# PathologyFoundation/plip

Measured on NVIDIA H100. Metric: image-text pairs/sec (224x224, 77-tok), higher is better.
Workload: dtype bf16

## Files before the change

plip_b200/csrc/attention.cu:

```cuda
#include <cfloat>

#include "kernels.cuh"
#include "wgmma.cuh"

namespace plip {

namespace {

constexpr int kAttThreads = 256;
constexpr uint32_t kTileBytes = 128 * 64 * 2;
constexpr uint32_t kStageBytes = 3 * kTileBytes;
constexpr uint32_t kAttSmem = kStageBytes + 1024 + 64;

__device__ __forceinline__ float fast_exp2(float x) {
  float y;
  asm("ex2.approx.ftz.f32 %0, %1;" : "=f"(y) : "f"(x));
  return y;
}
constexpr float kLog2e = 1.4426950408889634f;


template <bool F16, int NK>
__device__ __forceinline__ void qk_scores(float (&s)[NK / 2], uint64_t qdesc, uint64_t kdesc) {
  wgmma_pin(s);
  wgmma_fence();
#pragma unroll
  for (int k = 0; k < kHeadDim / 16; ++k) {
    if constexpr (NK == 64) wgmma_ss_n64<F16>(s, qdesc + 2 * k, kdesc + 2 * k, k != 0 ? 1u : 0u);
    else wgmma_ss_n128<F16>(s, qdesc + 2 * k, kdesc + 2 * k, k != 0 ? 1u : 0u);
  }
  wgmma_commit();
  wgmma_wait<0>();
  wgmma_pin(s);
}

__device__ __forceinline__ void quad_max(float& a, float& b) {
#pragma unroll
  for (int o = 1; o < 4; o <<= 1) {
    a = fmaxf(a, __shfl_xor_sync(0xffffffffu, a, o));
    b = fmaxf(b, __shfl_xor_sync(0xffffffffu, b, o));
  }
}
__device__ __forceinline__ void quad_sum(float& a, float& b) {
#pragma unroll
  for (int o = 1; o < 4; o <<= 1) {
    a += __shfl_xor_sync(0xffffffffu, a, o);
    b += __shfl_xor_sync(0xffffffffu, b, o);
  }
}

__device__ __forceinline__ int last_visible_key(int row, int S, int causal) {
  return row < S ? (causal ? row : S - 1) : -1;
}

template <int N>
__device__ __forceinline__ void mask_column(float (&s)[N], int j, int e, bool ok, int key, int lim0, int lim1) {
  if (!(ok && key <= lim0)) s[4 * j + e] = -INFINITY;
  if (!(ok && key <= lim1)) s[4 * j + 2 + e] = -INFINITY;
}

__device__ __forceinline__ float row_shift(float m) { return fmaxf(m * kLog2e, -FLT_MAX); }
__device__ __forceinline__ float row_inv(float l) { return l > 0.f ? 1.0f / l : 0.f; }

__device__ __forceinline__ float softmax_exp(float s, float ms) { return fast_exp2(fmaf(s, kLog2e, -ms)); }

__device__ __forceinline__ float2 fold_row_max(const float (&s)[32], float& m0, float& m1, float& l0, float& l1) {
  float mx0 = m0, mx1 = m1;
#pragma unroll
  for (int j = 0; j < 8; ++j) {
    mx0 = fmaxf(mx0, fmaxf(s[4 * j + 0], s[4 * j + 1]));
    mx1 = fmaxf(mx1, fmaxf(s[4 * j + 2], s[4 * j + 3]));
  }
  quad_max(mx0, mx1);
  const float alpha0 = softmax_exp(m0, row_shift(mx0)), alpha1 = softmax_exp(m1, row_shift(mx1));
  m0 = mx0;
  m1 = mx1;
  l0 *= alpha0;
  l1 *= alpha1;
  return make_float2(alpha0, alpha1);
}

template <bool F16, int N>
__device__ __forceinline__ void exp_sum_pack(const float (&s)[N], float ms0, float ms1, float& l0, float& l1,
                                             uint32_t (&pa)[N / 8][4]) {
#pragma unroll
  for (int j = 0; j < N / 4; ++j) {
    const float e00 = softmax_exp(s[4 * j + 0], ms0), e01 = softmax_exp(s[4 * j + 1], ms0);
    const float e10 = softmax_exp(s[4 * j + 2], ms1), e11 = softmax_exp(s[4 * j + 3], ms1);
    l0 += e00 + e01;
    l1 += e10 + e11;
    pa[j >> 1][2 * (j & 1) + 0] = pack_op2<F16>(e00, e01);
    pa[j >> 1][2 * (j & 1) + 1] = pack_op2<F16>(e10, e11);
  }
}

template <bool F16>
__device__ __forceinline__ void stage_rows(uint32_t row0, const float (&o)[32], float inv0, float inv1, int rr, int q4) {
  const uint32_t row1 = row0 + 8u * 128u;
#pragma unroll
  for (int j = 0; j < 8; ++j) {
    st_shared_b32(row0 + ((j ^ rr) << 4) + q4 * 4, pack_op2<F16>(o[4 * j + 0] * inv0, o[4 * j + 1] * inv0));
    st_shared_b32(row1 + ((j ^ rr) << 4) + q4 * 4, pack_op2<F16>(o[4 * j + 2] * inv1, o[4 * j + 3] * inv1));
  }
}

struct AttParams {
  int64_t n_seq;
  int seq_len;
  int slot;
  int group;
  int heads;
  int64_t seq_tiles;
  int causal;
  const int32_t* key_mask;
};

template <bool F16, int NK>
__global__ void __launch_bounds__(kAttThreads, NK == 64 ? 3 : 2)
attention_kernel(const __grid_constant__ CUtensorMap tmLoad, const __grid_constant__ CUtensorMap tmStore,
                 const AttParams p) {
  extern __shared__ uint8_t smem_raw[];
  const uint32_t smem_base = (smem_u32(smem_raw) + 1023u) & ~1023u;
  const uint32_t bar = smem_base + kStageBytes;
  const uint32_t sq = smem_base, sk = smem_base + kTileBytes, sv = smem_base + 2 * kTileBytes;

  const int warp = threadIdx.x >> 5;
  const int lane = threadIdx.x & 31;
  const int hf = warp >> 2;
  const int D = p.heads * kHeadDim;
  const int S = p.seq_len, G = p.group, slot = p.slot;

  if (threadIdx.x == 0) {
    tma_prefetch_desc(&tmLoad);
    tma_prefetch_desc(&tmStore);
    mbar_init(bar, 1);
    fence_mbar_init();
  }
  __syncthreads();

  const int ntiles = (int)(p.seq_tiles * p.heads);
  const uint32_t slot_bytes = static_cast<uint32_t>(slot) * 128u;
  auto issue_loads = [&](int tile) {
    const int64_t st = tile / p.heads;
    const int h = (int)(tile - st * p.heads);
    mbar_arrive_expect_tx(bar, 3 * kTileBytes);
    for (int g = 0; g < G; ++g) {
      const int32_t row = (int32_t)((st * G + g) * S);
      tma_load_2d(sq + g * slot_bytes, &tmLoad, bar, h * kHeadDim, row);
      tma_load_2d(sk + g * slot_bytes, &tmLoad, bar, D + h * kHeadDim, row);
      tma_load_2d(sv + g * slot_bytes, &tmLoad, bar, 2 * D + h * kHeadDim, row);
    }
  };
  if (threadIdx.x == 0 && (int)blockIdx.x < ntiles) issue_loads(blockIdx.x);

  const int q4 = lane & 3, rr = lane >> 2;
  const int R0 = 64 * hf + 16 * (warp & 3) + rr;
  const int g = R0 / slot;
  const int r_in0 = R0 - g * slot, r_in1 = r_in0 + 8;
  const int kbase = (NK == 64) ? 64 * hf : 0;
  const int k_in_base = kbase - g * slot + 2 * q4;
  const int lim0 = last_visible_key(r_in0, S, p.causal), lim1 = last_visible_key(r_in1, S, p.causal);

  uint32_t it = 0;
  for (int tile = blockIdx.x; tile < ntiles; tile += gridDim.x, ++it) {
    const int st = tile / p.heads;
    const int h = tile - st * p.heads;
    const int64_t seq = (int64_t)st * G + g;

    uint32_t kv = 0;
#pragma unroll
    for (int c = 0; c < NK / 4; ++c) {
      const int k_in = k_in_base + 8 * (c >> 1) + (c & 1);
      bool ok = k_in >= 0 && k_in < S;
      if (ok && p.key_mask != nullptr) ok = seq < p.n_seq && p.key_mask[seq * S + k_in] != 0;
      kv |= (ok ? 1u : 0u) << c;
    }

    mbar_wait(bar, it & 1u);

    float s[NK / 2];
    qk_scores<F16, NK>(s, make_smem_desc_sw128(sq + hf * (64 * 128), 1024, 16),
                       make_smem_desc_sw128(sk + kbase * 128, 1024, 16));

    float mx0 = -INFINITY, mx1 = -INFINITY;
#pragma unroll
    for (int c = 0; c < NK / 4; ++c) {
      const int j = c >> 1, e = c & 1;
      mask_column(s, j, e, (kv >> c) & 1u, k_in_base + 8 * j + e, lim0, lim1);
      mx0 = fmaxf(mx0, s[4 * j + e]);
      mx1 = fmaxf(mx1, s[4 * j + 2 + e]);
    }
    quad_max(mx0, mx1);
    float sum0 = 0.f, sum1 = 0.f;
    uint32_t pa[NK / 16][4];
    exp_sum_pack<F16>(s, row_shift(mx0), row_shift(mx1), sum0, sum1, pa);
    quad_sum(sum0, sum1);

    float o[32];
    wgmma_pin(o);
    wgmma_fence();
#pragma unroll
    for (int kk = 0; kk < NK / 16; ++kk) {
      const uint64_t vdesc = make_smem_desc_sw128(sv + (kbase + 16 * kk) * 128, 1024, 1024);
      wgmma_rs_n64<F16>(o, pa[kk], vdesc, kk != 0 ? 1u : 0u);
    }
    wgmma_commit();
    wgmma_wait<0>();
    wgmma_pin(o);

    stage_rows<F16>(sq + static_cast<uint32_t>(R0) * 128u, o, row_inv(sum0), row_inv(sum1), rr, q4);
    fence_proxy_async_smem();
    __syncthreads();
    if (threadIdx.x == 0) {
      for (int gg = 0; gg < G; ++gg) {
        const int64_t sq_idx = (int64_t)st * G + gg;
        if (sq_idx < p.n_seq)
          tma_store_2d(&tmStore, sq + static_cast<uint32_t>(gg * slot) * 128u, h * kHeadDim, (int32_t)(sq_idx * S));
      }
      tma_store_commit();
      tma_store_wait_read();
      if (tile + (int)gridDim.x < ntiles) issue_loads(tile + gridDim.x);
    }
  }
  if (threadIdx.x == 0) tma_store_wait_all();
}

template <bool F16, int NK>
int launch_attention_inst(const CUtensorMap& tmL, const CUtensorMap& tmS, const AttParams& p, cudaStream_t st) {
  auto kern = attention_kernel<F16, NK>;
  static unsigned long long configured = 0;
  static int grid_cap = 0;
  if (first_use_on_device(configured)) {
    PLIP_CUDA_CHECK(cudaFuncSetAttribute(kern, cudaFuncAttributeMaxDynamicSharedMemorySize, (int)kAttSmem));
    int dev = 0, sms = 0, per_sm = 0;
    PLIP_CUDA_CHECK(cudaGetDevice(&dev));
    PLIP_CUDA_CHECK(cudaDeviceGetAttribute(&sms, cudaDevAttrMultiProcessorCount, dev));
    PLIP_CUDA_CHECK(cudaOccupancyMaxActiveBlocksPerMultiprocessor(&per_sm, kern, kAttThreads, kAttSmem));
    grid_cap = (per_sm > 0 ? per_sm : 1) * sms;
  }
  const int64_t tiles = p.seq_tiles * p.heads;
  const int grid = (int)(tiles < grid_cap ? tiles : grid_cap);
  PLIP_CUDA_CHECK(launch_kernel(kern, dim3(grid), dim3(kAttThreads), kAttSmem, st, 1, tmL, tmS, p));
  return 0;
}

constexpr int kLongThreads = 288;
constexpr int kLongKeys = 64;
constexpr uint32_t kLongQBytes = 128 * 64 * 2;
constexpr uint32_t kLongKVBytes = kLongKeys * 64 * 2;
constexpr int kLongStages = 2;
constexpr uint32_t kLongSmem = kLongQBytes + kLongStages * 2 * kLongKVBytes + 1024 + 64;

struct LongAttParams {
  int seq_len;
  int heads;
  int q_blocks;
};

template <bool F16>
__global__ void __launch_bounds__(kLongThreads, 2)
attention_long_kernel(const __grid_constant__ CUtensorMap tmQKV, const __grid_constant__ CUtensorMap tmO,
                      const LongAttParams p) {
  extern __shared__ uint8_t smem_raw[];
  const uint32_t smem_base = (smem_u32(smem_raw) + 1023u) & ~1023u;
  const uint32_t sq = smem_base;
  auto sk = [&](int s) { return smem_base + kLongQBytes + (uint32_t)s * 2u * kLongKVBytes; };
  auto sv = [&](int s) { return sk(s) + kLongKVBytes; };
  const uint32_t bar = smem_base + kLongQBytes + kLongStages * 2 * kLongKVBytes;
  const uint32_t q_bar = bar;
  auto full_bar = [&](int s) { return bar + 8u * (1 + s); };
  auto empty_bar = [&](int s) { return bar + 8u * (1 + kLongStages + s); };

  const int warp = threadIdx.x >> 5;
  const int lane = threadIdx.x & 31;
  const int wg = warp >> 2;
  const int S = p.seq_len, D = p.heads * kHeadDim;
  const int qb = blockIdx.x % p.q_blocks;
  const int bh = blockIdx.x / p.q_blocks;
  const int h = bh % p.heads;
  const int seq = bh / p.heads;
  const int q0 = qb * 128;
  const int n_kb = (S + kLongKeys - 1) / kLongKeys;

  if (threadIdx.x == 0) {
    tma_prefetch_desc(&tmQKV);
    tma_prefetch_desc(&tmO);
    mbar_init(q_bar, 1);
    for (int s = 0; s < kLongStages; ++s) {
      mbar_init(full_bar(s), 1);
      mbar_init(empty_bar(s), 2);
    }
    fence_mbar_init();
  }
  __syncthreads();

  if (wg == 2) {
    if (lane == 0) {
      mbar_arrive_expect_tx(q_bar, kLongQBytes);
      tma_load_3d(sq, &tmQKV, q_bar, h * kHeadDim, q0, seq);
      tma_load_3d(sq + kLongQBytes / 2, &tmQKV, q_bar, h * kHeadDim, q0 + 64, seq);
      for (int kb = 0; kb < n_kb; ++kb) {
        const int s = kb % kLongStages;
        if (kb >= kLongStages) mbar_wait(empty_bar(s), (uint32_t)((kb / kLongStages - 1) & 1));
        mbar_arrive_expect_tx(full_bar(s), 2 * kLongKVBytes);
        tma_load_3d(sk(s), &tmQKV, full_bar(s), D + h * kHeadDim, kb * kLongKeys, seq);
        tma_load_3d(sv(s), &tmQKV, full_bar(s), 2 * D + h * kHeadDim, kb * kLongKeys, seq);
      }
    }
    return;
  }

  const int q4 = lane & 3, rr = lane >> 2;
  const int R0 = 64 * wg + 16 * (warp & 3) + rr;
  float o[32];
#pragma unroll
  for (int i = 0; i < 32; ++i) o[i] = 0.f;
  float m0 = -INFINITY, m1 = -INFINITY;
  float l0 = 0.f, l1 = 0.f;
  const uint64_t qdesc = make_smem_desc_sw128(sq + wg * (64 * 128), 1024, 16);
  mbar_wait(q_bar, 0);

  for (int kb = 0; kb < n_kb; ++kb) {
    const int s = kb % kLongStages;
    mbar_wait(full_bar(s), (uint32_t)((kb / kLongStages) & 1));

    float sc[32];
    qk_scores<F16, 64>(sc, qdesc, make_smem_desc_sw128(sk(s), 1024, 16));

    const int kbase = kb * kLongKeys + 2 * q4;
    if (kb * kLongKeys + kLongKeys > S) {
#pragma unroll
      for (int j = 0; j < 8; ++j)
#pragma unroll
        for (int e = 0; e < 2; ++e)
          if (kbase + 8 * j + e >= S) {
            sc[4 * j + e] = -INFINITY;
            sc[4 * j + 2 + e] = -INFINITY;
          }
    }
    const float2 alpha = fold_row_max(sc, m0, m1, l0, l1);
#pragma unroll
    for (int j = 0; j < 8; ++j) {
      o[4 * j + 0] *= alpha.x; o[4 * j + 1] *= alpha.x;
      o[4 * j + 2] *= alpha.y; o[4 * j + 3] *= alpha.y;
    }
    uint32_t pa[4][4];
    exp_sum_pack<F16>(sc, row_shift(m0), row_shift(m1), l0, l1, pa);

    wgmma_pin(o);
    wgmma_fence();
#pragma unroll
    for (int kk = 0; kk < kLongKeys / 16; ++kk) {
      const uint64_t vdesc = make_smem_desc_sw128(sv(s) + 16 * kk * 128, 1024, 1024);
      wgmma_rs_n64<F16>(o, pa[kk], vdesc, 1u);
    }
    wgmma_commit();
    wgmma_wait<0>();
    wgmma_pin(o);
    if ((threadIdx.x & 127) == 0) mbar_arrive(empty_bar(s));
  }

  quad_sum(l0, l1);
  stage_rows<F16>(sq + static_cast<uint32_t>(R0) * 128u, o, row_inv(l0), row_inv(l1), rr, q4);
  fence_proxy_async_smem();
  if (wg == 0) named_barrier_sync<1, 128>();
  else named_barrier_sync<2, 128>();
  if ((threadIdx.x & 127) == 0 && q0 + 64 * wg < S) {
    tma_store_3d(&tmO, sq + wg * (64 * 128), h * kHeadDim, q0 + 64 * wg, seq);
    tma_store_commit();
    tma_store_wait_all();
  }
}

constexpr int kProbThreads = 128;
constexpr int kProbStages = 2;
constexpr int kProbLd = 72;
constexpr uint32_t kProbTileBytes = 64 * 64 * 2;
constexpr uint32_t kProbStageOff = kProbTileBytes;
constexpr uint32_t kProbStagingOff = kProbStageOff + kProbStages * kProbTileBytes;
constexpr uint32_t kProbBarOff = kProbStagingOff + 64 * kProbLd * 4;
constexpr uint32_t kProbSmem = kProbBarOff + 8 * (1 + kProbStages) + 1024;

struct ProbParams {
  int seq_len;
  int heads;
  int q_blocks;
  int causal;
  const int32_t* key_mask;
  float* probs;
};

template <bool F16>
__global__ void __launch_bounds__(kProbThreads)
attention_probs_kernel(const __grid_constant__ CUtensorMap tmQKV, const ProbParams p) {
  extern __shared__ uint8_t smem_raw[];
  const uint32_t smem_base = (smem_u32(smem_raw) + 1023u) & ~1023u;
  float* staging = reinterpret_cast<float*>(smem_raw + (smem_base - smem_u32(smem_raw)) + kProbStagingOff);
  const uint32_t sq = smem_base;
  auto sk = [&](int s) { return smem_base + kProbStageOff + (uint32_t)s * kProbTileBytes; };
  const uint32_t q_bar = smem_base + kProbBarOff;
  auto full_bar = [&](int s) { return q_bar + 8u * (1 + s); };

  const int warp = threadIdx.x >> 5;
  const int lane = threadIdx.x & 31;
  const int S = p.seq_len, D = p.heads * kHeadDim;
  const int qb = blockIdx.x % p.q_blocks;
  const int64_t bh = blockIdx.x / p.q_blocks;
  const int h = (int)(bh % p.heads);
  const int64_t seq = bh / p.heads;
  const int q0 = qb * 64;
  const int n_kb = (S + 63) / 64;
  const bool resident = n_kb <= kProbStages;
  const int n_loads = resident ? n_kb : 2 * n_kb;

  auto issue_k = [&](int i) {
    const int s = i % kProbStages;
    mbar_arrive_expect_tx(full_bar(s), kProbTileBytes);
    tma_load_3d(sk(s), &tmQKV, full_bar(s), D + h * kHeadDim, (i % n_kb) * 64, (int32_t)seq);
  };
  if (threadIdx.x == 0) {
    tma_prefetch_desc(&tmQKV);
    mbar_init(q_bar, 1);
    for (int s = 0; s < kProbStages; ++s) mbar_init(full_bar(s), 1);
    fence_mbar_init();
    mbar_arrive_expect_tx(q_bar, kProbTileBytes);
    tma_load_3d(sq, &tmQKV, q_bar, h * kHeadDim, q0, (int32_t)seq);
    for (int i = 0; i < kProbStages && i < n_loads; ++i) issue_k(i);
  }
  __syncthreads();

  const int q4 = lane & 3, rr = lane >> 2;
  const int r0 = 16 * warp + rr;
  const int qa = q0 + r0, qc = qa + 8;
  const int lim0 = last_visible_key(qa, S, p.causal), lim1 = last_visible_key(qc, S, p.causal);
  const int32_t* km = p.key_mask ? p.key_mask + seq * S : nullptr;
  const uint64_t qdesc = make_smem_desc_sw128(sq, 1024, 16);
  mbar_wait(q_bar, 0);

  float sc[32];
  auto scores = [&](int u) {
    const int li = resident ? u % n_kb : u;
    const int s = li % kProbStages;
    mbar_wait(full_bar(s), (uint32_t)((li / kProbStages) & 1));
    qk_scores<F16, 64>(sc, qdesc, make_smem_desc_sw128(sk(s), 1024, 16));
    if (!resident) {
      __syncthreads();
      if (threadIdx.x == 0 && li + kProbStages < n_loads) issue_k(li + kProbStages);
    }
    const int kbase = (u % n_kb) * 64 + 2 * q4;
#pragma unroll
    for (int j = 0; j < 8; ++j)
#pragma unroll
      for (int e = 0; e < 2; ++e) {
        const int key = kbase + 8 * j + e;
        mask_column(sc, j, e, key < S && (km == nullptr || km[key] != 0), key, lim0, lim1);
      }
  };

  float m0 = -INFINITY, m1 = -INFINITY, l0 = 0.f, l1 = 0.f;
  for (int kb = 0; kb < n_kb; ++kb) {
    scores(kb);
    fold_row_max(sc, m0, m1, l0, l1);
    const float ms0 = row_shift(m0), ms1 = row_shift(m1);
#pragma unroll
    for (int j = 0; j < 8; ++j) {
      l0 += softmax_exp(sc[4 * j + 0], ms0) + softmax_exp(sc[4 * j + 1], ms0);
      l1 += softmax_exp(sc[4 * j + 2], ms1) + softmax_exp(sc[4 * j + 3], ms1);
    }
  }
  quad_sum(l0, l1);
  const float ms0 = row_shift(m0), ms1 = row_shift(m1);
  const float inv0 = row_inv(l0), inv1 = row_inv(l1);

  float* wst = staging + 16 * warp * kProbLd;
  const int rows = S - (q0 + 16 * warp) < 16 ? S - (q0 + 16 * warp) : 16;
  float* out_base = p.probs + ((seq * p.heads + h) * (int64_t)S + q0 + 16 * warp) * S;
  for (int kb = 0; kb < n_kb; ++kb) {
    scores(n_kb + kb);
#pragma unroll
    for (int j = 0; j < 8; ++j) {
      *reinterpret_cast<float2*>(wst + rr * kProbLd + 8 * j + 2 * q4) =
          make_float2(softmax_exp(sc[4 * j + 0], ms0) * inv0, softmax_exp(sc[4 * j + 1], ms0) * inv0);
      *reinterpret_cast<float2*>(wst + (rr + 8) * kProbLd + 8 * j + 2 * q4) =
          make_float2(softmax_exp(sc[4 * j + 2], ms1) * inv1, softmax_exp(sc[4 * j + 3], ms1) * inv1);
    }
    __syncwarp();
    const int k0 = kb * 64;
    const int nc = S - k0 < 64 ? S - k0 : 64;
    const int total = rows > 0 ? rows * nc : 0;
    int r = 0, c = lane;
    while (c >= nc) { c -= nc; ++r; }
    for (int i = lane; i < total; i += 32) {
      __stcs(out_base + (int64_t)r * S + k0 + c, wst[r * kProbLd + c]);
      c += 32;
      while (c >= nc) { c -= nc; ++r; }
    }
    __syncwarp();
  }
}

template <auto Kern, int Threads, uint32_t Smem, typename... Args>
int launch_blocks(int64_t blocks, cudaStream_t st, const Args&... args) {
  static unsigned long long configured = 0;
  if (first_use_on_device(configured))
    PLIP_CUDA_CHECK(cudaFuncSetAttribute(Kern, cudaFuncAttributeMaxDynamicSharedMemorySize, (int)Smem));
  PLIP_CUDA_CHECK(launch_kernel(Kern, dim3((unsigned)blocks), dim3(Threads), Smem, st, 1, args...));
  return 0;
}

int check_attention_args(const char* fn, const void* qkv, const void* out, int64_t n_seq, int seq_len, int heads) {
  PLIP_REQUIRE(qkv && out, "%s: null argument", fn);
  PLIP_REQUIRE(n_seq > 0 && seq_len > 0 && seq_len <= kMaxVisSeq, "%s: bad shape n_seq=%lld seq_len=%d", fn,
               (long long)n_seq, seq_len);
  PLIP_REQUIRE(heads > 0 && heads <= 16, "%s: bad head count %d", fn, heads);
  return 0;
}

int make_seq_tmap(CUtensorMap* tm, const void* base, int64_t n_seq, int seq_len, int cols) {
  return make_tmap_bf16_3d(tm, base, (uint64_t)n_seq, (uint64_t)seq_len, (uint64_t)cols, (uint64_t)cols * 2,
                           (uint64_t)seq_len * cols * 2, 64, 64);
}

}

int launch_attention(const __nv_bfloat16* qkv, int64_t n_seq, int seq_len, int heads, bool causal,
                     const int32_t* key_mask, __nv_bfloat16* out, int f16, cudaStream_t st) {
  if (int rc = check_attention_args("attention", qkv, out, n_seq, seq_len, heads)) return rc;
  const int D = heads * kHeadDim;
  if (seq_len > 128) {
    PLIP_REQUIRE(!causal && key_mask == nullptr,
                 "attention: seq_len %d > 128 is supported without causal or key mask only", seq_len);
    LongAttParams p;
    p.seq_len = seq_len;
    p.heads = heads;
    p.q_blocks = (seq_len + 127) / 128;
    const int64_t blocks = n_seq * heads * p.q_blocks;
    PLIP_REQUIRE(blocks < 0x7fffffff && n_seq < 0x7fffffff, "attention: too many sequences");
    CUtensorMap tmQKV, tmO;
    if (int rc = make_seq_tmap(&tmQKV, qkv, n_seq, seq_len, 3 * D)) return rc;
    if (int rc = make_seq_tmap(&tmO, out, n_seq, seq_len, D)) return rc;
    return f16 ? launch_blocks<attention_long_kernel<true>, kLongThreads, kLongSmem>(blocks, st, tmQKV, tmO, p)
               : launch_blocks<attention_long_kernel<false>, kLongThreads, kLongSmem>(blocks, st, tmQKV, tmO, p);
  }
  const int64_t rows = n_seq * seq_len;
  PLIP_REQUIRE(rows + 128 < 0x7fffffff, "attention: too many token rows");
  AttParams p;
  p.n_seq = n_seq;
  p.seq_len = seq_len;
  p.slot = seq_len <= 32 ? 32 : (seq_len <= 64 ? 64 : 128);
  p.group = 128 / p.slot;
  p.heads = heads;
  p.seq_tiles = (n_seq + p.group - 1) / p.group;
  p.causal = causal ? 1 : 0;
  p.key_mask = key_mask;
  CUtensorMap tmL, tmS;
  if (int rc = make_tmap_bf16_2d(&tmL, qkv, (uint64_t)rows, (uint64_t)3 * D, (uint64_t)3 * D * 2, (uint32_t)p.slot, 64)) return rc;
  if (int rc = make_tmap_bf16_2d(&tmS, out, (uint64_t)rows, (uint64_t)D, (uint64_t)D * 2, (uint32_t)seq_len, 64)) return rc;
  PLIP_REQUIRE(p.seq_tiles * heads < 0x7fffffff, "attention: too many tiles");
  if (p.slot == 128) return f16 ? launch_attention_inst<true, 128>(tmL, tmS, p, st) : launch_attention_inst<false, 128>(tmL, tmS, p, st);
  return f16 ? launch_attention_inst<true, 64>(tmL, tmS, p, st) : launch_attention_inst<false, 64>(tmL, tmS, p, st);
}

int launch_attention_probs(const __nv_bfloat16* qkv, int64_t n_seq, int seq_len, int heads, bool causal,
                           const int32_t* key_mask, float* probs, int f16, cudaStream_t st) {
  if (int rc = check_attention_args("attention_probs", qkv, probs, n_seq, seq_len, heads)) return rc;
  ProbParams p;
  p.seq_len = seq_len;
  p.heads = heads;
  p.q_blocks = (seq_len + 63) / 64;
  p.causal = causal ? 1 : 0;
  p.key_mask = key_mask;
  p.probs = probs;
  const int64_t blocks = n_seq * heads * p.q_blocks;
  PLIP_REQUIRE(blocks < 0x7fffffff && n_seq < 0x7fffffff, "attention_probs: too many sequences");
  const int D = heads * kHeadDim;
  CUtensorMap tm;
  if (int rc = make_seq_tmap(&tm, qkv, n_seq, seq_len, 3 * D)) return rc;
  return f16 ? launch_blocks<attention_probs_kernel<true>, kProbThreads, kProbSmem>(blocks, st, tm, p)
             : launch_blocks<attention_probs_kernel<false>, kProbThreads, kProbSmem>(blocks, st, tm, p);
}

}
```

Measured before the change: 27780.

## Restructure short-sequence attention into per-head 64-row blocks using 3D TMA

Replaces the packed-slot short attention kernel (which grouped several sequences into a 128-row tile with masks, and for seq 65-128 computed a full 128-key n128 QK tile) with a unit-based kernel. For seq_len ≤64 each warpgroup handles a separate (sequence, head) item, and for seq_len 65-128 the two warpgroups split the query rows, processing one or two 64-key blocks (only one below the diagonal when causal). Loads use 3D per-sequence tensor maps, so TMA zero-fills padding rather than loading neighbouring sequences. This is meant to cut wasted masked compute and cross-sequence masking overhead. In exchange it adds branches on the number of key blocks and more register arrays.

```diff
diff --git a/plip_b200/csrc/attention.cu b/plip_b200/csrc/attention.cu
--- a/plip_b200/csrc/attention.cu
+++ b/plip_b200/csrc/attention.cu
@@ -8,9 +8,9 @@
 namespace {
 
 constexpr int kAttThreads = 256;
-constexpr uint32_t kTileBytes = 128 * 64 * 2;
-constexpr uint32_t kStageBytes = 3 * kTileBytes;
-constexpr uint32_t kAttSmem = kStageBytes + 1024 + 64;
+constexpr uint32_t kBlockBytes = 64 * 64 * 2;
+constexpr uint32_t kAttOperandBytes = 6 * kBlockBytes;
+constexpr uint32_t kAttSmem = kAttOperandBytes + 1024 + 64;
 
 __device__ __forceinline__ float fast_exp2(float x) {
   float y;
@@ -20,15 +20,12 @@
 constexpr float kLog2e = 1.4426950408889634f;
 
 
-template <bool F16, int NK>
-__device__ __forceinline__ void qk_scores(float (&s)[NK / 2], uint64_t qdesc, uint64_t kdesc) {
+template <bool F16>
+__device__ __forceinline__ void qk_scores(float (&s)[32], uint64_t qdesc, uint64_t kdesc) {
   wgmma_pin(s);
   wgmma_fence();
 #pragma unroll
-  for (int k = 0; k < kHeadDim / 16; ++k) {
-    if constexpr (NK == 64) wgmma_ss_n64<F16>(s, qdesc + 2 * k, kdesc + 2 * k, k != 0 ? 1u : 0u);
-    else wgmma_ss_n128<F16>(s, qdesc + 2 * k, kdesc + 2 * k, k != 0 ? 1u : 0u);
-  }
+  for (int k = 0; k < kHeadDim / 16; ++k) wgmma_ss_n64<F16>(s, qdesc + 2 * k, kdesc + 2 * k, k != 0 ? 1u : 0u);
   wgmma_commit();
   wgmma_wait<0>();
   wgmma_pin(s);
@@ -64,13 +61,17 @@
 
 __device__ __forceinline__ float softmax_exp(float s, float ms) { return fast_exp2(fmaf(s, kLog2e, -ms)); }
 
-__device__ __forceinline__ float2 fold_row_max(const float (&s)[32], float& m0, float& m1, float& l0, float& l1) {
-  float mx0 = m0, mx1 = m1;
+__device__ __forceinline__ void thread_row_max(const float (&s)[32], float& mx0, float& mx1) {
 #pragma unroll
   for (int j = 0; j < 8; ++j) {
     mx0 = fmaxf(mx0, fmaxf(s[4 * j + 0], s[4 * j + 1]));
     mx1 = fmaxf(mx1, fmaxf(s[4 * j + 2], s[4 * j + 3]));
   }
+}
+
+__device__ __forceinline__ float2 fold_row_max(const float (&s)[32], float& m0, float& m1, float& l0, float& l1) {
+  float mx0 = m0, mx1 = m1;
+  thread_row_max(s, mx0, mx1);
   quad_max(mx0, mx1);
   const float alpha0 = softmax_exp(m0, row_shift(mx0)), alpha1 = softmax_exp(m1, row_shift(mx1));
   m0 = mx0;
@@ -104,130 +105,146 @@
   }
 }
 
+template <bool F16>
+__device__ __forceinline__ void masked_scores(float (&s)[32], uint64_t qdesc, uint32_t kblock, uint32_t kv, int key0,
+                                              int lim0, int lim1) {
+  qk_scores<F16>(s, qdesc, make_smem_desc_sw128(kblock, 1024, 16));
+#pragma unroll
+  for (int c = 0; c < 16; ++c) {
+    const int j = c >> 1, e = c & 1;
+    mask_column(s, j, e, (kv >> c) & 1u, key0 + 8 * j + e, lim0, lim1);
+  }
+}
+
 struct AttParams {
-  int64_t n_seq;
   int seq_len;
-  int slot;
-  int group;
   int heads;
-  int64_t seq_tiles;
+  int items;
+  int units;
   int causal;
   const int32_t* key_mask;
 };
 
-template <bool F16, int NK>
-__global__ void __launch_bounds__(kAttThreads, NK == 64 ? 3 : 2)
-attention_kernel(const __grid_constant__ CUtensorMap tmLoad, const __grid_constant__ CUtensorMap tmStore,
+template <bool F16, bool SPLIT>
+__global__ void __launch_bounds__(kAttThreads, SPLIT ? 2 : 3)
+attention_kernel(const __grid_constant__ CUtensorMap tmQKV, const __grid_constant__ CUtensorMap tmO,
                  const AttParams p) {
   extern __shared__ uint8_t smem_raw[];
   const uint32_t smem_base = (smem_u32(smem_raw) + 1023u) & ~1023u;
-  const uint32_t bar = smem_base + kStageBytes;
-  const uint32_t sq = smem_base, sk = smem_base + kTileBytes, sv = smem_base + 2 * kTileBytes;
+  const uint32_t sq = smem_base, sk = sq + 2 * kBlockBytes, sv = sk + 2 * kBlockBytes;
+  const uint32_t bar = smem_base + kAttOperandBytes;
 
   const int warp = threadIdx.x >> 5;
   const int lane = threadIdx.x & 31;
-  const int hf = warp >> 2;
-  const int D = p.heads * kHeadDim;
-  const int S = p.seq_len, G = p.group, slot = p.slot;
+  const int wg = warp >> 2;
+  const int S = p.seq_len, D = p.heads * kHeadDim;
+  constexpr bool split = SPLIT;
 
   if (threadIdx.x == 0) {
-    tma_prefetch_desc(&tmLoad);
-    tma_prefetch_desc(&tmStore);
+    tma_prefetch_desc(&tmQKV);
+    tma_prefetch_desc(&tmO);
     mbar_init(bar, 1);
     fence_mbar_init();
   }
   __syncthreads();
 
-  const int ntiles = (int)(p.seq_tiles * p.heads);
-  const uint32_t slot_bytes = static_cast<uint32_t>(slot) * 128u;
-  auto issue_loads = [&](int tile) {
-    const int64_t st = tile / p.heads;
-    const int h = (int)(tile - st * p.heads);
-    mbar_arrive_expect_tx(bar, 3 * kTileBytes);
-    for (int g = 0; g < G; ++g) {
-      const int32_t row = (int32_t)((st * G + g) * S);
-      tma_load_2d(sq + g * slot_bytes, &tmLoad, bar, h * kHeadDim, row);
-      tma_load_2d(sk + g * slot_bytes, &tmLoad, bar, D + h * kHeadDim, row);
-      tma_load_2d(sv + g * slot_bytes, &tmLoad, bar, 2 * D + h * kHeadDim, row);
+  auto item_of = [&](int u, int t) { return split ? u : 2 * u + t; };
+  auto issue_loads = [&](int u) {
+    const int nb = item_of(u, 1) < p.items ? 2 : 1;
+    mbar_arrive_expect_tx(bar, nb * 3 * kBlockBytes);
+    for (int t = 0; t < nb; ++t) {
+      const int it = item_of(u, t);
+      const int seq = it / p.heads, row = split ? 64 * t : 0;
+      const int c = (it - seq * p.heads) * kHeadDim;
+      tma_load_3d(sq + t * kBlockBytes, &tmQKV, bar, c, row, seq);
+      tma_load_3d(sk + t * kBlockBytes, &tmQKV, bar, D + c, row, seq);
+      tma_load_3d(sv + t * kBlockBytes, &tmQKV, bar, 2 * D + c, row, seq);
     }
   };
-  if (threadIdx.x == 0 && (int)blockIdx.x < ntiles) issue_loads(blockIdx.x);
+  if (threadIdx.x == 0 && (int)blockIdx.x < p.units) issue_loads(blockIdx.x);
 
   const int q4 = lane & 3, rr = lane >> 2;
-  const int R0 = 64 * hf + 16 * (warp & 3) + rr;
-  const int g = R0 / slot;
-  const int r_in0 = R0 - g * slot, r_in1 = r_in0 + 8;
-  const int kbase = (NK == 64) ? 64 * hf : 0;
-  const int k_in_base = kbase - g * slot + 2 * q4;
-  const int lim0 = last_visible_key(r_in0, S, p.causal), lim1 = last_visible_key(r_in1, S, p.causal);
-
-  uint32_t it = 0;
-  for (int tile = blockIdx.x; tile < ntiles; tile += gridDim.x, ++it) {
-    const int st = tile / p.heads;
-    const int h = tile - st * p.heads;
-    const int64_t seq = (int64_t)st * G + g;
+  const int r0 = 16 * (warp & 3) + rr;
+  const int qa = split ? 64 * wg + r0 : r0;
+  const int lim0 = last_visible_key(qa, S, p.causal), lim1 = last_visible_key(qa + 8, S, p.causal);
+  const int kb0 = split ? 0 : wg;
+  const int nkb = split ? (p.causal ? wg + 1 : 2) : 1;
+  const uint64_t qdesc = make_smem_desc_sw128(sq + wg * kBlockBytes, 1024, 16);
+
+  uint32_t iter = 0;
+  for (int u = blockIdx.x; u < p.units; u += gridDim.x, ++iter) {
+    const int item = item_of(u, wg);
+    const bool active = item < p.items;
+    const int64_t seq = item / p.heads;
 
     uint32_t kv = 0;
 #pragma unroll
-    for (int c = 0; c < NK / 4; ++c) {
-      const int k_in = k_in_base + 8 * (c >> 1) + (c & 1);
-      bool ok = k_in >= 0 && k_in < S;
-      if (ok && p.key_mask != nullptr) ok = seq < p.n_seq && p.key_mask[seq * S + k_in] != 0;
-      kv |= (ok ? 1u : 0u) << c;
-    }
-
-    mbar_wait(bar, it & 1u);
-
-    float s[NK / 2];
-    qk_scores<F16, NK>(s, make_smem_desc_sw128(sq + hf * (64 * 128), 1024, 16),
-                       make_smem_desc_sw128(sk + kbase * 128, 1024, 16));
-
-    float mx0 = -INFINITY, mx1 = -INFINITY;
-#pragma unroll
-    for (int c = 0; c < NK / 4; ++c) {
-      const int j = c >> 1, e = c & 1;
-      mask_column(s, j, e, (kv >> c) & 1u, k_in_base + 8 * j + e, lim0, lim1);
-      mx0 = fmaxf(mx0, s[4 * j + e]);
-      mx1 = fmaxf(mx1, s[4 * j + 2 + e]);
-    }
-    quad_max(mx0, mx1);
-    float sum0 = 0.f, sum1 = 0.f;
-    uint32_t pa[NK / 16][4];
-    exp_sum_pack<F16>(s, row_shift(mx0), row_shift(mx1), sum0, sum1, pa);
-    quad_sum(sum0, sum1);
-
-    float o[32];
-    wgmma_pin(o);
-    wgmma_fence();
-#pragma unroll
-    for (int kk = 0; kk < NK / 16; ++kk) {
-      const uint64_t vdesc = make_smem_desc_sw128(sv + (kbase + 16 * kk) * 128, 1024, 1024);
-      wgmma_rs_n64<F16>(o, pa[kk], vdesc, kk != 0 ? 1u : 0u);
-    }
-    wgmma_commit();
-    wgmma_wait<0>();
-    wgmma_pin(o);
-
-    stage_rows<F16>(sq + static_cast<uint32_t>(R0) * 128u, o, row_inv(sum0), row_inv(sum1), rr, q4);
-    fence_proxy_async_smem();
+    for (int b = 0; b < 2; ++b)
+#pragma unroll
+      for (int c = 0; c < 16; ++c) {
+        const int key = 64 * b + 8 * (c >> 1) + 2 * q4 + (c & 1);
+        bool ok = b < nkb && key < S;
+        if (ok && p.key_mask != nullptr) ok = active && p.key_mask[seq * S + key] != 0;
+        kv |= (ok ? 1u : 0u) << (16 * b + c);
+      }
+
+    mbar_wait(bar, iter & 1u);
+
+    if (active) {
+      float s[32];
+      float mx0 = -INFINITY, mx1 = -INFINITY;
+      float l0 = 0.f, l1 = 0.f;
+      uint32_t pa0[4][4], pa1[4][4];
+      masked_scores<F16>(s, qdesc, sk + kb0 * kBlockBytes, kv, 2 * q4, lim0, lim1);
+      thread_row_max(s, mx0, mx1);
+      if (nkb == 2) {
+        float s1[32];
+        masked_scores<F16>(s1, qdesc, sk + (kb0 + 1) * kBlockBytes, kv >> 16, 64 + 2 * q4, lim0, lim1);
+        thread_row_max(s1, mx0, mx1);
+        quad_max(mx0, mx1);
+        exp_sum_pack<F16>(s, row_shift(mx0), row_shift(mx1), l0, l1, pa0);
+        exp_sum_pack<F16>(s1, row_shift(mx0), row_shift(mx1), l0, l1, pa1);
+      } else {
+        quad_max(mx0, mx1);
+        exp_sum_pack<F16>(s, row_shift(mx0), row_shift(mx1), l0, l1, pa0);
+      }
+
+      float o[32];
+      wgmma_pin(o);
+      wgmma_fence();
+#pragma unroll
+      for (int kk = 0; kk < 8; ++kk) {
+        if (kk == 4 * nkb) break;
+        const uint64_t vdesc = make_smem_desc_sw128(sv + kb0 * kBlockBytes + 16 * kk * 128, 1024, 1024);
+        wgmma_rs_n64<F16>(o, kk < 4 ? pa0[kk] : pa1[kk - 4], vdesc, kk != 0 ? 1u : 0u);
+      }
+      wgmma_commit();
+      wgmma_wait<0>();
+      wgmma_pin(o);
+      quad_sum(l0, l1);
+
+      stage_rows<F16>(sq + wg * kBlockBytes + static_cast<uint32_t>(r0) * 128u, o, row_inv(l0), row_inv(l1), rr, q4);
+      fence_proxy_async_smem();
+    }
     __syncthreads();
     if (threadIdx.x == 0) {
-      for (int gg = 0; gg < G; ++gg) {
-        const int64_t sq_idx = (int64_t)st * G + gg;
-        if (sq_idx < p.n_seq)
-          tma_store_2d(&tmStore, sq + static_cast<uint32_t>(gg * slot) * 128u, h * kHeadDim, (int32_t)(sq_idx * S));
+      for (int t = 0; t < 2; ++t) {
+        const int it = item_of(u, t);
+        if (it >= p.items) break;
+        const int sseq = it / p.heads;
+        tma_store_3d(&tmO, sq + t * kBlockBytes, (it - sseq * p.heads) * kHeadDim, split ? 64 * t : 0, sseq);
       }
       tma_store_commit();
       tma_store_wait_read();
-      if (tile + (int)gridDim.x < ntiles) issue_loads(tile + gridDim.x);
+      if (u + (int)gridDim.x < p.units) issue_loads(u + gridDim.x);
     }
   }
   if (threadIdx.x == 0) tma_store_wait_all();
 }
 
-template <bool F16, int NK>
-int launch_attention_inst(const CUtensorMap& tmL, const CUtensorMap& tmS, const AttParams& p, cudaStream_t st) {
-  auto kern = attention_kernel<F16, NK>;
+template <bool F16, bool SPLIT>
+int launch_attention_short(const CUtensorMap& tmQKV, const CUtensorMap& tmO, const AttParams& p, cudaStream_t st) {
+  auto kern = attention_kernel<F16, SPLIT>;
   static unsigned long long configured = 0;
   static int grid_cap = 0;
   if (first_use_on_device(configured)) {
@@ -238,9 +255,8 @@
     PLIP_CUDA_CHECK(cudaOccupancyMaxActiveBlocksPerMultiprocessor(&per_sm, kern, kAttThreads, kAttSmem));
     grid_cap = (per_sm > 0 ? per_sm : 1) * sms;
   }
-  const int64_t tiles = p.seq_tiles * p.heads;
-  const int grid = (int)(tiles < grid_cap ? tiles : grid_cap);
-  PLIP_CUDA_CHECK(launch_kernel(kern, dim3(grid), dim3(kAttThreads), kAttSmem, st, 1, tmL, tmS, p));
+  const int grid = (int)(p.units < grid_cap ? p.units : grid_cap);
+  PLIP_CUDA_CHECK(launch_kernel(kern, dim3(grid), dim3(kAttThreads), kAttSmem, st, 1, tmQKV, tmO, p));
   return 0;
 }
 
@@ -325,7 +341,7 @@
     mbar_wait(full_bar(s), (uint32_t)((kb / kLongStages) & 1));
 
     float sc[32];
-    qk_scores<F16, 64>(sc, qdesc, make_smem_desc_sw128(sk(s), 1024, 16));
+    qk_scores<F16>(sc, qdesc, make_smem_desc_sw128(sk(s), 1024, 16));
 
     const int kbase = kb * kLongKeys + 2 * q4;
     if (kb * kLongKeys + kLongKeys > S) {
@@ -442,7 +458,7 @@
     const int li = resident ? u % n_kb : u;
     const int s = li % kProbStages;
     mbar_wait(full_bar(s), (uint32_t)((li / kProbStages) & 1));
-    qk_scores<F16, 64>(sc, qdesc, make_smem_desc_sw128(sk(s), 1024, 16));
+    qk_scores<F16>(sc, qdesc, make_smem_desc_sw128(sk(s), 1024, 16));
     if (!resident) {
       __syncthreads();
       if (threadIdx.x == 0 && li + kProbStages < n_loads) issue_k(li + kProbStages);
@@ -526,39 +542,34 @@
 int launch_attention(const __nv_bfloat16* qkv, int64_t n_seq, int seq_len, int heads, bool causal,
                      const int32_t* key_mask, __nv_bfloat16* out, int f16, cudaStream_t st) {
   if (int rc = check_attention_args("attention", qkv, out, n_seq, seq_len, heads)) return rc;
+  PLIP_REQUIRE(n_seq < 0x7fffffff, "attention: too many sequences");
+  PLIP_REQUIRE(seq_len <= 128 || (!causal && key_mask == nullptr),
+               "attention: seq_len %d > 128 is supported without causal or key mask only", seq_len);
   const int D = heads * kHeadDim;
+  CUtensorMap tmQKV, tmO;
+  if (int rc = make_seq_tmap(&tmQKV, qkv, n_seq, seq_len, 3 * D)) return rc;
+  if (int rc = make_seq_tmap(&tmO, out, n_seq, seq_len, D)) return rc;
   if (seq_len > 128) {
-    PLIP_REQUIRE(!causal && key_mask == nullptr,
-                 "attention: seq_len %d > 128 is supported without causal or key mask only", seq_len);
     LongAttParams p;
     p.seq_len = seq_len;
     p.heads = heads;
     p.q_blocks = (seq_len + 127) / 128;
     const int64_t blocks = n_seq * heads * p.q_blocks;
-    PLIP_REQUIRE(blocks < 0x7fffffff && n_seq < 0x7fffffff, "attention: too many sequences");
-    CUtensorMap tmQKV, tmO;
-    if (int rc = make_seq_tmap(&tmQKV, qkv, n_seq, seq_len, 3 * D)) return rc;
-    if (int rc = make_seq_tmap(&tmO, out, n_seq, seq_len, D)) return rc;
+    PLIP_REQUIRE(blocks < 0x7fffffff, "attention: too many sequences");
     return f16 ? launch_blocks<attention_long_kernel<true>, kLongThreads, kLongSmem>(blocks, st, tmQKV, tmO, p)
                : launch_blocks<attention_long_kernel<false>, kLongThreads, kLongSmem>(blocks, st, tmQKV, tmO, p);
   }
-  const int64_t rows = n_seq * seq_len;
-  PLIP_REQUIRE(rows + 128 < 0x7fffffff, "attention: too many token rows");
+  PLIP_REQUIRE(n_seq * heads < 0x7fffffff, "attention: too many sequences");
   AttParams p;
-  p.n_seq = n_seq;
   p.seq_len = seq_len;
-  p.slot = seq_len <= 32 ? 32 : (seq_len <= 64 ? 64 : 128);
-  p.group = 128 / p.slot;
   p.heads = heads;
-  p.seq_tiles = (n_seq + p.group - 1) / p.group;
+  p.items = (int)(n_seq * heads);
+  p.units = seq_len > 64 ? p.items : p.items / 2 + (p.items & 1);
   p.causal = causal ? 1 : 0;
   p.key_mask = key_mask;
-  CUtensorMap tmL, tmS;
-  if (int rc = make_tmap_bf16_2d(&tmL, qkv, (uint64_t)rows, (uint64_t)3 * D, (uint64_t)3 * D * 2, (uint32_t)p.slot, 64)) return rc;
-  if (int rc = make_tmap_bf16_2d(&tmS, out, (uint64_t)rows, (uint64_t)D, (uint64_t)D * 2, (uint32_t)seq_len, 64)) return rc;
-  PLIP_REQUIRE(p.seq_tiles * heads < 0x7fffffff, "attention: too many tiles");
-  if (p.slot == 128) return f16 ? launch_attention_inst<true, 128>(tmL, tmS, p, st) : launch_attention_inst<false, 128>(tmL, tmS, p, st);
-  return f16 ? launch_attention_inst<true, 64>(tmL, tmS, p, st) : launch_attention_inst<false, 64>(tmL, tmS, p, st);
+  if (seq_len > 64)
+    return f16 ? launch_attention_short<true, true>(tmQKV, tmO, p, st) : launch_attention_short<false, true>(tmQKV, tmO, p, st);
+  return f16 ? launch_attention_short<true, false>(tmQKV, tmO, p, st) : launch_attention_short<false, false>(tmQKV, tmO, p, st);
 }
 
 int launch_attention_probs(const __nv_bfloat16* qkv, int64_t n_seq, int seq_len, int heads, bool causal,
```

After: 27970, median of 6. About the same (+0.7%).
